# Aatricks/LightDiffusion-Next

Measured on AMD Instinct MI355X. Metric: sampler it/s (UNet steps/sec) SD1.5 1024x1024 bs=1 bf16, higher is better.
Workload: dtype bf16

## Files before the change

include/ldx.h:

```cpp
#ifndef LDX_H
#define LDX_H
#include <stdint.h>
#ifdef __cplusplus
extern "C" {
#endif

#define LDX_OK 0
#define LDX_EINVAL (-1)
#define LDX_EMISSING (-2)
#define LDX_EHIP (-3)
#define LDX_ESTATE (-4)

#define LDX_BF16 0
#define LDX_F16 1
#define LDX_F32 2

typedef struct ldx_engine ldx_engine;

typedef struct ldx_unet_config {
    int32_t compute_dtype;
    int32_t in_channels;
    int32_t out_channels;
    int32_t model_channels;
    int32_t num_levels;
// ... 139 lines not shown
int ldx_op_mx_quant(const void* X, int ldx, int rows, int K, void* Y, int ldy, void* scales, int scales_ld, int dtype, void* stream);
int ldx_op_gemm_mx(const void* A8, int lda, const void* SA, int sa_ld, const void* W8, const void* SW, int sw_ld, int M, int N, int K,
                   const float* bias, int act, const void* R, int ldr, void* C, int ldc, float* Cf, int ldcf,
                   void* C8, int ldc8, void* SC, int sc_ld, int dtype, void* stream);
int ldx_op_gemm2(const void* A1, int lda1, const void* W1, int M1, int N1, int K1, const float* bias1, void* C1, int ldc1,
                 const void* A2, int lda2, const void* W2, int M2, int N2, int K2, const float* bias2, void* C2, int ldc2, int dtype, void* stream);
int ldx_op_gemm2_mx(const void* A1, int lda1, const void* SA1, int sa_ld1, const void* W1, const void* SW1, int sw_ld1, int M1, int N1, int K1,
                    const float* bias1, void* C1, int ldc1,
                    const void* A2, int lda2, const void* SA2, int sa_ld2, const void* W2, const void* SW2, int sw_ld2, int M2, int N2, int K2,
                    const float* bias2, void* C2, int ldc2, int dtype, void* stream);
int ldx_op_gemm_pick(int M, int N, int K, int mode, int geglu, int splitk, int f8, int c8, int ln_fold,
                     int Cin, int Hin, int Win, int Hout, int Wout, int stride, int M2, int N2, int K2,
                     int gn_hw, int gn_groups, int gn_max_chunks, int32_t* out);
int ldx_op_attn_pick(int B, int H, int Nq, int Mk, int D, int causal, int bias, int o8, int ldq, int ldk, int ldv, int ldo, int knorm_ws, int32_t* out);
int ldx_op_conv3x3(const void* X, int ldx, const void* W, int B, int Hin, int Win, int Cin, int Cout,
                   int stride, int Hout, int Wout, int resize_to_out, const float* bias,
                   const float* rowvec, int rowvec_ld, const void* R, int ldr, void* Y, int ldy,
                   int dtype, void* stream);
int ldx_op_conv3x3_skip(const void* X, int ldx, const void* X2, int ldx2, int Cin2, const void* W, int B, int H, int Wd, int Cin, int Cout,
                        const float* bias, void* Y, int ldy, int dtype, void* stream);
int ldx_op_groupnorm(const void* X, int ldx, void* Y, int ldy, int B, int HW, int C, int G, float eps, int silu,
                     const float* gamma, const float* beta, float* workspace, int dtype, void* stream);
int64_t ldx_op_groupnorm_workspace_floats(int B, int G);
int ldx_op_layernorm(const void* X, int ldx, void* Y, int ldy, int rows, int C, float eps,
                     const float* gamma, const float* beta, int dtype, void* stream);
int ldx_op_attention(const void* Q, int ldq, const void* K, int ldk, const void* V, int ldv, void* O, int ldo,
                     int B, int H, int Nq, int Mk, int D, float scale, int causal, int dtype, void* stream);
int ldx_op_xattn_block(void* H, int ldh, int64_t M, int N, int C, int heads, const float* ln_gamma, const float* ln_beta, float eps,
                       const void* Wq, const void* Wo, const float* bo, const void* K, int ldk, const void* V, int ldv, int Mk,
                       float scale, int dtype, void* stream);
int ldx_op_ff_block(void* H, int ldh, int64_t M, int C, int inner, const float* ln_gamma, const float* ln_beta, float eps,
                    const void* W1, const float* b1, const void* W2, const float* b2, int dtype, void* stream);
int ldx_op_rowgemm(const void* X, int ldx, void* Y, int ldy, int64_t M, int N, int K, const void* W, const float* bias, const void* R, int ldr,
                   int pro, const float* gamma, const float* beta, float eps, const float* partial, int nchunk, int HW, int dtype, void* stream);
int ldx_op_attention_bias(const void* Q, int ldq, const void* K, int ldk, const void* V, int ldv, void* O, int ldo,
                          int B, int H, int Nq, int Mk, int D, float scale, const float* bias, int bias_ld,
                          int64_t bias_head_stride, int dtype, void* stream);
int ldx_op_skinny(const float* x, int ldx, const void* W, const float* bias, float* out, int ldo,
                  int M, int N, int K, int in_act, int out_act, int dtype, void* stream);

#ifdef __cplusplus
}
#endif
#endif
```

lightdiffusion-next_amd/csrc/capi.cpp:

```cpp
#include <cstring>
#include <mutex>
#include <new>

#include "engine.h"

using namespace ldx;

struct ldx_engine { Engine* impl; };

#define GUARD_BEGIN try {
#define GUARD_END                                                                  \
    }                                                                              \
    catch (const std::bad_alloc&) { set_error("out of host memory"); return LDX_EINVAL; } \
    catch (const std::exception& ex) { set_error(std::string("internal error: ") + ex.what()); return LDX_EINVAL; }

static int check_device(int device) {
    int n = 0;
    if (hipGetDeviceCount(&n) != hipSuccess || n <= 0) { set_error("no HIP device available (libldx has no CPU fallback)"); return LDX_EHIP; }
    if (device < 0 || device >= n) { set_error("device ordinal out of range"); return LDX_EINVAL; }
    return LDX_OK;
}
static inline DType dtype_of(int d) { return d == LDX_F16 ? DT_F16 : DT_BF16; }
static int check_launch(const char* what) {
    hipError_t e = hipGetLastError();
// ... 515 lines not shown
    return check_launch("ldx_op_conv3x3");
}
int ldx_op_conv3x3_skip(const void* X, int ldx_, const void* X2, int ldx2, int Cin2, const void* W, int B, int H, int Wd, int Cin, int Cout,
                        const float* bias, void* Y, int ldy, int dtype, void* stream) {
    if (!X || !X2 || !W || !Y || Cin % 64 || Cin2 % 64 || ldx_ % 8 || ldx2 % 8 || B <= 0 || H <= 0 || Wd <= 0) {
        set_error("ldx_op_conv3x3_skip: bad argument (Cin % 64, Cin2 % 64)"); return LDX_EINVAL; }
    GemmArgs g{};
    g.A = X; g.lda = ldx_; g.W = W; g.M = B * H * Wd; g.N = Cout; g.K = 9 * Cin + Cin2; g.mode = 1;
    g.Cin = Cin; g.Hin = H; g.Win = Wd; g.Hout = H; g.Wout = Wd; g.stride = 1; g.Hv = H; g.Wv = Wd; g.resize = 0;
    g.A2 = X2; g.lda2 = ldx2; g.Cin2 = Cin2;
    g.bias = bias; g.rows_per_batch = H * Wd; g.C = Y; g.ldc = ldy;
    if (int rc = attach_splitk(g)) return rc;
    launch_gemm(g, dtype_of(dtype), (hipStream_t)stream);
    return check_launch("ldx_op_conv3x3_skip");
}
int64_t ldx_op_groupnorm_workspace_floats(int B, int G) { return (int64_t)B * GN_NCHUNK * G * 2; }
int ldx_op_groupnorm(const void* X, int ldx_, void* Y, int ldy, int B, int HW, int C, int G, float eps, int silu,
                     const float* gamma, const float* beta, float* workspace, int dtype, void* stream) {
    if (!X || !Y || !gamma || !beta || !workspace || C % 8 || C % G || G > 32 || ldx_ % 8 || ldy % 8) { set_error("ldx_op_groupnorm: bad argument"); return LDX_EINVAL; }
    GroupNormArgs a{X, ldx_, Y, ldy, B, HW, C, G, eps, silu, gamma, beta, workspace};
    launch_groupnorm(a, dtype_of(dtype), (hipStream_t)stream);
    return check_launch("ldx_op_groupnorm");
}
int ldx_op_layernorm(const void* X, int ldx_, void* Y, int ldy, int rows, int C, float eps, const float* gamma, const float* beta, int dtype, void* stream) {
    if (!X || !Y || !gamma || !beta || C % 8 || C > 4096) { set_error("ldx_op_layernorm: bad argument (C % 8, C <= 4096)"); return LDX_EINVAL; }
    LayerNormArgs a{X, ldx_, Y, ldy, rows, C, eps, gamma, beta};
    launch_layernorm(a, dtype_of(dtype), (hipStream_t)stream);
    return check_launch("ldx_op_layernorm");
}
int ldx_op_attention(const void* Q, int ldq, const void* K, int ldk, const void* V, int ldv, void* O, int ldo, int B, int H, int Nq, int Mk, int D,
                     float scale, int causal, int dtype, void* stream) {
    if (!Q || !K || !V || !O || D % 8 || (D > 160 && D != 512) || D <= 0 || ldq % 8 || ldk % 8 || ldv % 8 || ldo % 4 || Mk <= 0) { set_error("ldx_op_attention: bad argument (D % 8, D <= 160 or D == 512)"); return LDX_EINVAL; }
    AttnArgs a{Q, ldq, K, ldk, V, ldv, O, ldo, B, H, Nq, Mk, D, scale, causal, nullptr, 0, 0};
    const AttnPick p = attn_pick(a);
    if (D == 512 && p.family != AF_ATTN512) { set_error("ldx_op_attention: D = 512 without a mask only (attn512.hip)"); return LDX_EINVAL; }
    if (p.nsplit_want > 1) {
        a.nsplit = p.nsplit_want;
        a.split_ws = op_workspace(attn512_ws_floats(a, a.nsplit));
        if (!a.split_ws) { set_error("attention split workspace allocation failed"); return LDX_EHIP; }
    }
    if (attn_pipe_ok(a)) a.knorm_ws = op_workspace((size_t)B * H * ((Mk + 63) / 64));
    launch_attention(a, dtype_of(dtype), (hipStream_t)stream);
    return check_launch("ldx_op_attention");
}
int ldx_op_xattn_block(void* H, int ldh, int64_t M, int N, int C, int heads, const float* ln_gamma, const float* ln_beta, float eps,
                       const void* Wq, const void* Wo, const float* bo, const void* K, int ldk, const void* V, int ldv, int Mk,
// ... 45 lines not shown
```

lightdiffusion-next_amd/csrc/ldx_kernels.h:

```cpp
#pragma once
#include <hip/hip_runtime.h>
#include <stdint.h>

namespace ldx {

enum DType : int { DT_BF16 = 0, DT_F16 = 1 };

struct DevOnce { unsigned long long mask = 0; };
inline void set_dyn_lds(DevOnce& once, const void* fn, int bytes) {
    int dev = 0;
    (void)hipGetDevice(&dev);
    const unsigned long long bit = 1ull << (dev & 63);
    if (__atomic_load_n(&once.mask, __ATOMIC_RELAXED) & bit) return;
    (void)hipFuncSetAttribute(fn, hipFuncAttributeMaxDynamicSharedMemorySize, bytes);
    __atomic_fetch_or(&once.mask, bit, __ATOMIC_RELAXED);
}

struct GemmArgs {
    const void* A;  int lda;
    const void* W;
    int M, N, K;
    int mode;
    int Cin, Hin, Win;
    int Hv, Wv;
// ... 117 lines not shown
    float* gn_out; int gn_nchunk;
    int abl;
    long dup_rows;
};
bool rowgemm_ok(const RowGemmArgs& a);
void launch_rowgemm(const RowGemmArgs& a, DType dt, hipStream_t s);
bool xattn_block_ok(const XAttnArgs& a);
void launch_xattn_block(const XAttnArgs& a, DType dt, hipStream_t s);

struct GroupNormArgs {
    const void* X; int ldx; void* Y; int ldy;
    int B, HW, C, G; float eps; int silu;
    const float* gamma; const float* beta;
    float* partial;
    int nchunk;
    int stats_chunks;
};
constexpr int GN_NCHUNK = 256;
constexpr int GN_FOLD = 64;
constexpr int GN_MAX_PRODUCER_CHUNKS = 32768;
static inline size_t gn_workspace_rows(long HWmax) { long r = HWmax / 64; if (r < GN_NCHUNK) r = GN_NCHUNK; if (r > GN_MAX_PRODUCER_CHUNKS) r = GN_MAX_PRODUCER_CHUNKS; return (size_t)r; }
void launch_groupnorm(const GroupNormArgs& a, DType dt, hipStream_t s);
bool gn_uses_small_kernel(int B, long HW, int C, int G);

struct LayerNormArgs {
    const void* X; int ldx; void* Y; int ldy; int rows, C; float eps;
    const float* gamma; const float* beta;
    const float* scale; const float* shift; int mod_ld; int rows_per_batch;
    int rms;
    void* Y8; int ldy8; uint32_t* S8; int s8_ld;
};
void launch_layernorm(const LayerNormArgs& a, DType dt, hipStream_t s);

struct PrepArgs {
    const float* x; const float* sigma; int B, C, H, W; int Cpad; void* xc;
    const float* log_sigmas; int n_sigmas; const float* temb_table; int temb_dim;
    float* temb_out; float* t_out;
    int scale_input;
    const float* t_in;
    int xB;
    const float* cc; int Cx;
    const float* emb_table; int emb_n; float* emb_out;
};
void launch_prep(const PrepArgs& a, DType dt, hipStream_t s);
void launch_timestep(const float* sigma, const float* log_sigmas, int n_sigmas, int n, int* out, hipStream_t s);
struct FinishArgs { const float* eps; int ld; const float* x; const float* sigma; float* out; int B, C, HW; int xB; };
// ... 61 lines not shown
```

lightdiffusion-next_amd/csrc/norm.hip:

```cpp
#include <stdlib.h>
#include "ldx_device.h"
#include "ldx_kernels.h"

namespace ldx {

struct GnGeom { int CH, TX, RY; };
static inline GnGeom gn_geom(int C) {
    const int cpp = C / 8;
    int ch = 1;
    while (ch < 4 && (cpp / ch > 256 || cpp % ch)) ch *= 2;
    GnGeom g; g.CH = ch; g.TX = cpp / ch; g.RY = 256 / g.TX; if (g.RY < 1) g.RY = 1;
    return g;
}

template <typename T, int CH>
__global__ __launch_bounds__(256) void gn_stats_kernel(const GroupNormArgs p, int TX, int RY) {
    extern __shared__ float sred[];
    const int tid = threadIdx.x;
    const int tx = tid % TX, ty = tid / TX;
    const int b = blockIdx.y, chunk = blockIdx.x;
    const int per = (p.HW + p.nchunk - 1) / p.nchunk;
    const int pb = chunk * per, pe = min(p.HW, pb + per);
    const T* __restrict__ X = (const T*)p.X + (long)b * p.HW * p.ldx;

    float s[CH][8], q[CH][8];
#pragma unroll
    for (int k = 0; k < CH; ++k)
#pragma unroll
        for (int e = 0; e < 8; ++e) { s[k][e] = 0.f; q[k][e] = 0.f; }

    if (ty < RY) {
        int pix = pb + ty;
        for (; pix + 3 * RY < pe; pix += 4 * RY) {
            uint4 u[4][CH];
#pragma unroll
            for (int r = 0; r < 4; ++r)
#pragma unroll
                for (int k = 0; k < CH; ++k) u[r][k] = *(const uint4*)(X + (long)(pix + r * RY) * p.ldx + (tx + TX * k) * 8);
#pragma unroll
            for (int r = 0; r < 4; ++r)
#pragma unroll
                for (int k = 0; k < CH; ++k) {
                    float f[8];
                    unpack8<T>(u[r][k], f);
#pragma unroll
                    for (int e = 0; e < 8; ++e) { s[k][e] += f[e]; q[k][e] = fmaf(f[e], f[e], q[k][e]); }
                }
        }
        for (; pix < pe; pix += RY) {
#pragma unroll
            for (int k = 0; k < CH; ++k) {
                float f[8];
                unpack8<T>(*(const uint4*)(X + (long)pix * p.ldx + (tx + TX * k) * 8), f);
#pragma unroll
                for (int e = 0; e < 8; ++e) { s[k][e] += f[e]; q[k][e] = fmaf(f[e], f[e], q[k][e]); }
            }
        }
#pragma unroll
        for (int k = 0; k < CH; ++k)
#pragma unroll
            for (int e = 0; e < 8; ++e) {
                const int c = (tx + TX * k) * 8 + e;
                sred[(ty * p.C + c) * 2 + 0] = s[k][e];
                sred[(ty * p.C + c) * 2 + 1] = q[k][e];
            }
    }
    __syncthreads();
    if (tid < p.G * 2) {
        const int g = tid >> 1, st = tid & 1;
        const int cpg = p.C / p.G;
        float acc = 0.f;
        for (int r = 0; r < RY; ++r)
            for (int c = g * cpg; c < (g + 1) * cpg; ++c) acc += sred[(r * p.C + c) * 2 + st];
        p.partial[(((long)b * p.nchunk + chunk) * p.G + g) * 2 + st] = acc;
    }
}

template <typename T, int CH>
__global__ __launch_bounds__(256) void gn_apply_kernel(const GroupNormArgs p, int TX, int RY, int nblk) {
    __shared__ float smean[64], srstd[64];
    __shared__ float sred[8][32][2];
    const int tid = threadIdx.x;
    const int b = blockIdx.y;
    const int cpg = p.C / p.G;
    const int tx = tid % TX, ty = tid / TX;
    const bool act = ty < RY;
    const T* __restrict__ X = (const T*)p.X + (long)b * p.HW * p.ldx;
    T* __restrict__ Y = (T*)p.Y + (long)b * p.HW * p.ldy;
    const int per = (p.HW + nblk - 1) / nblk;
    const int pb = blockIdx.x * per, pe = min(p.HW, pb + per);
    int pix = pb + ty;
    uint4 u0[4][CH];
    const bool first4 = act && pix + 3 * RY < pe;
    if (first4) {
#pragma unroll
        for (int r = 0; r < 4; ++r)
#pragma unroll
            for (int k = 0; k < CH; ++k) u0[r][k] = *(const uint4*)(X + (long)(pix + r * RY) * p.ldx + (tx + TX * k) * 8);
    }
    float4 gam[CH][2], bet[CH][2];
    if (act) {
#pragma unroll
        for (int k = 0; k < CH; ++k) {
            const int c = (tx + TX * k) * 8;
            gam[k][0] = *(const float4*)(p.gamma + c); gam[k][1] = *(const float4*)(p.gamma + c + 4);
            bet[k][0] = *(const float4*)(p.beta + c);  bet[k][1] = *(const float4*)(p.beta + c + 4);
        }
    }
    {
        const int g = tid & 31, sl = tid >> 5;
        float su = 0.f, sq = 0.f;
        if (g < p.G) {
            const float2* pp = (const float2*)p.partial + ((long)b * p.nchunk) * p.G + g;
            int ck = sl;
            for (; ck + 120 < p.nchunk; ck += 128) {
                float2 v[16];
#pragma unroll
                for (int u = 0; u < 16; ++u) v[u] = pp[(long)(ck + 8 * u) * p.G];
#pragma unroll
                for (int u = 0; u < 16; ++u) { su += v[u].x; sq += v[u].y; }
            }
            for (; ck + 56 < p.nchunk; ck += 64) {
                float2 v[8];
#pragma unroll
                for (int u = 0; u < 8; ++u) v[u] = pp[(long)(ck + 8 * u) * p.G];
#pragma unroll
                for (int u = 0; u < 8; ++u) { su += v[u].x; sq += v[u].y; }
            }
            for (; ck < p.nchunk; ck += 8) { const float2 v = pp[(long)ck * p.G]; su += v.x; sq += v.y; }
        }
        sred[sl][g][0] = su; sred[sl][g][1] = sq;
    }
    __syncthreads();
    if (tid < p.G) {
        float su = 0.f, sq = 0.f;
#pragma unroll
        for (int sl = 0; sl < 8; ++sl) { su += sred[sl][tid][0]; sq += sred[sl][tid][1]; }
        const float n = (float)p.HW * (float)cpg;
        const float mean = su / n;
        const float var = fmaxf(sq / n - mean * mean, 0.f);
        smean[tid] = mean;
        srstd[tid] = rsqrtf(var + p.eps);
    }
    __syncthreads();
    if (!act) return;
    float sc[CH][8], sh[CH][8];
#pragma unroll
    for (int k = 0; k < CH; ++k) {
        const float ga[8] = {gam[k][0].x, gam[k][0].y, gam[k][0].z, gam[k][0].w, gam[k][1].x, gam[k][1].y, gam[k][1].z, gam[k][1].w};
        const float be[8] = {bet[k][0].x, bet[k][0].y, bet[k][0].z, bet[k][0].w, bet[k][1].x, bet[k][1].y, bet[k][1].z, bet[k][1].w};
#pragma unroll
        for (int e = 0; e < 8; ++e) {
            const int c = (tx + TX * k) * 8 + e;
            const int g = c / cpg;
            const float a = srstd[g] * ga[e];
            sc[k][e] = a;
            sh[k][e] = be[e] - smean[g] * a;
        }
    }
    auto emit = [&](const uint4& u, const int pix, const int k) __attribute__((always_inline)) {
        float f[8];
        unpack8<T>(u, f);
#pragma unroll
        for (int e = 0; e < 8; ++e) {
            float y = fmaf(f[e], sc[k][e], sh[k][e]);
            if (p.silu) y = silu_f(y);
            f[e] = y;
        }
        *(uint4*)(Y + (long)pix * p.ldy + (tx + TX * k) * 8) = pack8<T>(f);
    };
    if (first4) {
#pragma unroll
        for (int r = 0; r < 4; ++r)
#pragma unroll
            for (int k = 0; k < CH; ++k) emit(u0[r][k], pix + r * RY, k);
        pix += 4 * RY;
    }
    for (; pix + 3 * RY < pe; pix += 4 * RY) {
        uint4 u[4][CH];
#pragma unroll
        for (int r = 0; r < 4; ++r)
#pragma unroll
            for (int k = 0; k < CH; ++k) u[r][k] = *(const uint4*)(X + (long)(pix + r * RY) * p.ldx + (tx + TX * k) * 8);
#pragma unroll
        for (int r = 0; r < 4; ++r)
#pragma unroll
            for (int k = 0; k < CH; ++k) emit(u[r][k], pix + r * RY, k);
    }
    for (; pix < pe; pix += RY) {
#pragma unroll
        for (int k = 0; k < CH; ++k) emit(*(const uint4*)(X + (long)pix * p.ldx + (tx + TX * k) * 8), pix, k);
    }
}

template <typename T>
__global__ __launch_bounds__(256) void gn_small_kernel(const GroupNormArgs p) {
    __shared__ float red[2][4];
    const int tid = threadIdx.x, g = blockIdx.x, b = blockIdx.y;
    const int cpg = p.C / p.G, cpc = cpg >> 3;
    const long total = (long)p.HW * cpc;
    const T* __restrict__ X = (const T*)p.X + (long)b * p.HW * p.ldx + g * cpg;
    T* __restrict__ Y = (T*)p.Y + (long)b * p.HW * p.ldy + g * cpg;
    float su = 0.f, sq = 0.f;
    constexpr int KMAX = 12;
    if (total <= (long)KMAX * 256) {
        uint4 u[KMAX]; int px[KMAX], cc[KMAX];
#pragma unroll
        for (int k = 0; k < KMAX; ++k) {
            const long ii = (long)tid + 256 * k;
            px[k] = (int)(ii / cpc); cc[k] = (int)(ii % cpc);
            u[k] = ii < total ? *(const uint4*)(X + (long)px[k] * p.ldx + cc[k] * 8) : make_uint4(0u, 0u, 0u, 0u);
        }
#pragma unroll
        for (int k = 0; k < KMAX; ++k) {
            if ((long)tid + 256 * k < total) {
                float f[8];
                unpack8<T>(u[k], f);
#pragma unroll
                for (int e = 0; e < 8; ++e) { su += f[e]; sq = fmaf(f[e], f[e], sq); }
            }
        }
        su = wave_sum(su); sq = wave_sum(sq);
        if ((tid & 63) == 0) { red[0][tid >> 6] = su; red[1][tid >> 6] = sq; }
        __syncthreads();
        const float n = (float)p.HW * (float)cpg;
        const float mean = ((red[0][0] + red[0][1]) + (red[0][2] + red[0][3])) / n;
        const float var = fmaxf(((red[1][0] + red[1][1]) + (red[1][2] + red[1][3])) / n - mean * mean, 0.f);
        const float rstd = rsqrtf(var + p.eps);
#pragma unroll
        for (int k = 0; k < KMAX; ++k) {
            if ((long)tid + 256 * k < total) {
                float f[8];
                unpack8<T>(u[k], f);
                const float* gm = p.gamma + g * cpg + cc[k] * 8;
                const float* bt = p.beta + g * cpg + cc[k] * 8;
                const float4 g0 = *(const float4*)gm, g1 = *(const float4*)(gm + 4), b0 = *(const float4*)bt, b1 = *(const float4*)(bt + 4);
                const float gg[8] = {g0.x, g0.y, g0.z, g0.w, g1.x, g1.y, g1.z, g1.w}, bb[8] = {b0.x, b0.y, b0.z, b0.w, b1.x, b1.y, b1.z, b1.w};
#pragma unroll
                for (int e = 0; e < 8; ++e) {
                    const float a = rstd * gg[e];
                    float y = fmaf(f[e], a, bb[e] - mean * a);
                    if (p.silu) y = silu_f(y);
                    f[e] = y;
                }
                *(uint4*)(Y + (long)px[k] * p.ldy + cc[k] * 8) = pack8<T>(f);
            }
        }
        return;
    }
    long i = tid;
    for (; i + 3 * 256 < total; i += 4 * 256) {
        uint4 u[4];
#pragma unroll
        for (int r = 0; r < 4; ++r) {
            const long ii = i + r * 256;
            const int pix = (int)(ii / cpc), ch = (int)(ii % cpc);
            u[r] = *(const uint4*)(X + (long)pix * p.ldx + ch * 8);
        }
#pragma unroll
        for (int r = 0; r < 4; ++r) {
            float f[8];
            unpack8<T>(u[r], f);
#pragma unroll
            for (int e = 0; e < 8; ++e) { su += f[e]; sq = fmaf(f[e], f[e], sq); }
        }
    }
    for (; i < total; i += 256) {
        const int pix = (int)(i / cpc), ch = (int)(i % cpc);
        float f[8];
        unpack8<T>(*(const uint4*)(X + (long)pix * p.ldx + ch * 8), f);
#pragma unroll
        for (int e = 0; e < 8; ++e) { su += f[e]; sq = fmaf(f[e], f[e], sq); }
    }
    su = wave_sum(su); sq = wave_sum(sq);
    if ((tid & 63) == 0) { red[0][tid >> 6] = su; red[1][tid >> 6] = sq; }
    __syncthreads();
    const float n = (float)p.HW * (float)cpg;
    const float mean = ((red[0][0] + red[0][1]) + (red[0][2] + red[0][3])) / n;
    const float var = fmaxf(((red[1][0] + red[1][1]) + (red[1][2] + red[1][3])) / n - mean * mean, 0.f);
    const float rstd = rsqrtf(var + p.eps);
    auto emit = [&](const uint4& u, const int pix, const int ch) __attribute__((always_inline)) {
        float f[8];
        unpack8<T>(u, f);
        const float* gm = p.gamma + g * cpg + ch * 8;
        const float* bt = p.beta + g * cpg + ch * 8;
        const float4 g0 = *(const float4*)gm, g1 = *(const float4*)(gm + 4), b0 = *(const float4*)bt, b1 = *(const float4*)(bt + 4);
        const float gg[8] = {g0.x, g0.y, g0.z, g0.w, g1.x, g1.y, g1.z, g1.w}, bb[8] = {b0.x, b0.y, b0.z, b0.w, b1.x, b1.y, b1.z, b1.w};
#pragma unroll
        for (int e = 0; e < 8; ++e) {
            const float a = rstd * gg[e];
            float y = fmaf(f[e], a, bb[e] - mean * a);
            if (p.silu) y = silu_f(y);
            f[e] = y;
        }
        *(uint4*)(Y + (long)pix * p.ldy + ch * 8) = pack8<T>(f);
    };
    i = tid;
    for (; i + 3 * 256 < total; i += 4 * 256) {
        uint4 u[4]; int px[4], cc[4];
#pragma unroll
        for (int r = 0; r < 4; ++r) {
            const long ii = i + r * 256;
            px[r] = (int)(ii / cpc); cc[r] = (int)(ii % cpc);
            u[r] = *(const uint4*)(X + (long)px[r] * p.ldx + cc[r] * 8);
        }
#pragma unroll
        for (int r = 0; r < 4; ++r) emit(u[r], px[r], cc[r]);
    }
    for (; i < total; i += 256) {
        const int pix = (int)(i / cpc), ch = (int)(i % cpc);
// ... 2 lines not shown
}

__global__ __launch_bounds__(64) void gn_fold_kernel(const float* in, float* out, int n_in, int G) {
    const int f = blockIdx.x, b = blockIdx.y, t = threadIdx.x;
    if (t >= G * 2) return;
    const int per = (n_in + GN_FOLD - 1) / GN_FOLD;
    const int lo = f * per, hi = min(n_in, lo + per);
    float a0 = 0.f, a1 = 0.f, a2 = 0.f, a3 = 0.f;
    int c = lo;
    for (; c + 3 < hi; c += 4) {
        const float v0 = in[((long)b * n_in + c) * G * 2 + t], v1 = in[((long)b * n_in + c + 1) * G * 2 + t];
        const float v2 = in[((long)b * n_in + c + 2) * G * 2 + t], v3 = in[((long)b * n_in + c + 3) * G * 2 + t];
        a0 += v0; a1 += v1; a2 += v2; a3 += v3;
    }
    for (; c < hi; ++c) a0 += in[((long)b * n_in + c) * G * 2 + t];
    out[((long)b * GN_FOLD + f) * G * 2 + t] = (a0 + a1) + (a2 + a3);
}

bool gn_uses_small_kernel(int B, long HW, int C, int G) {
    static const long small_max = getenv("LDX_GN_SMALL_MAX") ? atol(getenv("LDX_GN_SMALL_MAX")) : 256 * 80;
    return G > 0 && (C / G) % 8 == 0 && HW * (C / G) <= small_max && (long)G * B >= 32;
}

template <typename T>
static void launch_gn_t(const GroupNormArgs& a_in, hipStream_t s) {
    GroupNormArgs a = a_in;
    if (a.stats_chunks > 0) {
        const GnGeom g = gn_geom(a.C);
        a.nchunk = a.stats_chunks;
        if (a.stats_chunks > GN_NCHUNK) {
            float* folded = a.partial + (size_t)a.B * a.stats_chunks * a.G * 2;
            hipLaunchKernelGGL(gn_fold_kernel, dim3(GN_FOLD, a.B), dim3(64), 0, s, a.partial, folded, a.stats_chunks, a.G);
            a.partial = folded; a.nchunk = GN_FOLD;
        }
        int nblk = (a.HW + g.RY * 8 - 1) / (g.RY * 8);
        if (nblk > 512) nblk = 512;
        if (nblk < 1) nblk = 1;
        dim3 grid2(nblk, a.B);
        switch (g.CH) {
            case 1: hipLaunchKernelGGL((gn_apply_kernel<T, 1>), grid2, dim3(256), 0, s, a, g.TX, g.RY, nblk); break;
            case 2: hipLaunchKernelGGL((gn_apply_kernel<T, 2>), grid2, dim3(256), 0, s, a, g.TX, g.RY, nblk); break;
            default: hipLaunchKernelGGL((gn_apply_kernel<T, 4>), grid2, dim3(256), 0, s, a, g.TX, g.RY, nblk); break;
        }
        return;
    }
    if (gn_uses_small_kernel(a.B, a.HW, a.C, a.G)) {
        hipLaunchKernelGGL((gn_small_kernel<T>), dim3(a.G, a.B), dim3(256), 0, s, a);
        return;
    }
    const GnGeom g = gn_geom(a.C);
    int nchunk = (1024 + a.B - 1) / a.B;
    const int maxc = (a.HW + g.RY * 4 - 1) / (g.RY * 4);
    if (nchunk > maxc) nchunk = maxc;
    if (nchunk > GN_NCHUNK) nchunk = GN_NCHUNK;
    if (nchunk < 1) nchunk = 1;
    a.nchunk = nchunk;
    dim3 grid1(nchunk, a.B);
    const size_t lds = (size_t)g.RY * a.C * 2 * sizeof(float);
    int nblk = (a.HW + g.RY * 8 - 1) / (g.RY * 8);
    if (nblk > 512) nblk = 512;
    if (nblk < 1) nblk = 1;
    dim3 grid2(nblk, a.B);
    switch (g.CH) {
        case 1:
            hipLaunchKernelGGL((gn_stats_kernel<T, 1>), grid1, dim3(256), lds, s, a, g.TX, g.RY);
            hipLaunchKernelGGL((gn_apply_kernel<T, 1>), grid2, dim3(256), 0, s, a, g.TX, g.RY, nblk);
            break;
        case 2:
            hipLaunchKernelGGL((gn_stats_kernel<T, 2>), grid1, dim3(256), lds, s, a, g.TX, g.RY);
            hipLaunchKernelGGL((gn_apply_kernel<T, 2>), grid2, dim3(256), 0, s, a, g.TX, g.RY, nblk);
            break;
        default:
            hipLaunchKernelGGL((gn_stats_kernel<T, 4>), grid1, dim3(256), lds, s, a, g.TX, g.RY);
            hipLaunchKernelGGL((gn_apply_kernel<T, 4>), grid2, dim3(256), 0, s, a, g.TX, g.RY, nblk);
            break;
    }
}

void launch_groupnorm(const GroupNormArgs& a, DType dt, hipStream_t s) {
    if (dt == DT_BF16) launch_gn_t<__bf16>(a, s); else launch_gn_t<_Float16>(a, s);
}

template <typename T, int LPR, int NCH>
__global__ __launch_bounds__(256) void ln_kernel(const LayerNormArgs p) {
    constexpr int RPW = 64 / LPR;
    const int lane = threadIdx.x & 63, sub = lane % LPR;
    const long row_raw = ((long)blockIdx.x * 4 + (threadIdx.x >> 6)) * RPW + lane / LPR;
    const bool live = row_raw < p.rows;
    const long row = live ? row_raw : p.rows - 1;
    const int nch = p.C >> 3;
    const T* __restrict__ x = (const T*)p.X + row * p.ldx;
    T* __restrict__ y = (T*)p.Y + row * p.ldy;
    float f[NCH][8];
    float sum = 0.f;
    uint4 raw[NCH];
#pragma unroll
    for (int i = 0; i < NCH; ++i) { const int ch = sub + LPR * i; raw[i] = *(const uint4*)(x + (ch < nch ? ch : 0) * 8); }
#pragma unroll
    for (int i = 0; i < NCH; ++i) {
// ... 124 lines not shown
```

lightdiffusion-next_amd/lib.py:

```python
import ctypes as C
import os

_HERE = os.path.dirname(os.path.abspath(__file__))
LIB_PATH = os.path.join(_HERE, "libldx.so")

LDX_BF16, LDX_F16, LDX_F32 = 0, 1, 2


class LdxError(RuntimeError):
    pass


class ldx_unet_config(C.Structure):
    _fields_ = [
        ("compute_dtype", C.c_int32),
        ("in_channels", C.c_int32),
        ("out_channels", C.c_int32),
        ("model_channels", C.c_int32),
        ("num_levels", C.c_int32),
        ("channel_mult", C.c_int32 * 8),
        ("num_res_blocks", C.c_int32 * 8),
        ("transformer_depth", C.c_int32 * 32),
        ("transformer_depth_output", C.c_int32 * 48),
        ("transformer_depth_middle", C.c_int32),
# ... 59 lines not shown
    "ldx_clip_encode": (_i, [_vp, _vp, _i, _i, _i, _vp, _vp, _vp]),
    "ldx_clip_pooled": (_i, [_vp, _vp, _vp, _i, _i, _i, _vp, _vp]),
    "ldx_clip_set_extra_embeddings": (_i, [_vp, _vp, _i]),
    "ldx_flux_fbcache": (_i, [_vp, _f]),
    "ldx_flux_set_fp8": (_i, [_vp, _i]),
    "ldx_flux_fbcache_stats": (_i, [_vp, C.POINTER(_i64), C.POINTER(_i64)]),
    "ldx_esrgan_create": (_i, [C.POINTER(ldx_esrgan_config), _i, C.POINTER(_vp)]),
    "ldx_esrgan_forward": (_i, [_vp, _vp, _i, _i, _i, _vp, _vp]),
    "ldx_tile_blend": (_i, [_vp, _i, _i, _vp, _vp, _i, _i, _i, _i, _i, _i, _vp]),
    "ldx_tile_finish": (_i, [_vp, _vp, _i64, _i, _vp]),
    "ldx_t5_create": (_i, [C.POINTER(ldx_t5_config), _i, C.POINTER(_vp)]),
    "ldx_t5_encode": (_i, [_vp, _vp, _i, _i, _vp, _vp, _vp]),
    "ldx_flux_create": (_i, [C.POINTER(ldx_flux_config), _i, C.POINTER(_vp)]),
    "ldx_flux_forward": (_i, [_vp, _vp, _vp, _vp, _vp, _vp, _vp, _vp, _i, _i, _i, _i, _i, _vp, _vp]),
    "ldx_sampler_step": (_i, [_i, _vp, _vp, _vp, _vp, _i64, _f, _f, _f, _vp]),
    "ldx_bislerp_pass": (_i, [_vp, _vp, _i, _i, _i, _i, _i, _i, _vp, _vp, _vp, _vp]),
    "ldx_vae_encode": (_i, [_vp, _vp, _i, _i, _i, _vp, _vp]),
    "ldx_bilinear": (_i, [_vp, _vp, _i, _i, _i, _i, _i, _vp]),
    "ldx_op_convert": (_i, [_vp, _vp, _i64, _i, _i, _vp]),
    "ldx_op_gemm": (_i, [_vp, _i, _vp, _i, _i, _i, _vp, _vp, _i, _i, _i, _vp, _i, _vp, _i, _vp, _i, _i, _vp]),
    "ldx_op_conv3x3": (_i, [_vp, _i, _vp, _i, _i, _i, _i, _i, _i, _i, _i, _i, _vp, _vp, _i, _vp, _i, _vp, _i, _i, _vp]),
    "ldx_op_groupnorm": (_i, [_vp, _i, _vp, _i, _i, _i, _i, _i, _f, _i, _vp, _vp, _vp, _i, _vp]),
    "ldx_op_groupnorm_workspace_floats": (_i64, [_i, _i]),
    "ldx_op_conv3x3_skip": (_i, [_vp, _i, _vp, _i, _i, _vp, _i, _i, _i, _i, _i, _vp, _vp, _i, _i, _vp]),
    "ldx_op_layernorm_mx": (_i, [_vp, _i, _i, _i, _f, _vp, _vp, _vp, _i, _vp, _i, _i, _vp]),
    "ldx_op_attention_mx": (_i, [_vp, _i, _vp, _i, _vp, _i, _vp, _i, _vp, _i, _i, _i, _i, _i, _f, _i, _vp]),
    "ldx_op_qk_norm_rope_mx": (_i, [_vp, _i, _i, _i, _i, _vp, _vp, _vp, _vp, _f, _vp, _vp, _i, _vp, _vp, _i, _i, _vp]),
    "ldx_op_mx_vt_quant": (_i, [_vp, _i, _i, _i, _i, _vp, _vp, _i, _i, _vp]),
    "ldx_op_attention_fp8": (_i, [_vp, _i, _vp, _i, _vp, _i, _vp, _i, _vp, _vp, _i, _vp, _i, _vp, _i, _vp, _i, _i, _i, _i, _i, _f, _i, _vp]),
    "ldx_op_mx_quant": (_i, [_vp, _i, _i, _i, _vp, _i, _vp, _i, _i, _vp]),
    "ldx_op_gemm2": (_i, [_vp, _i, _vp, _i, _i, _i, _vp, _vp, _i, _vp, _i, _vp, _i, _i, _i, _vp, _vp, _i, _i, _vp]),
    "ldx_op_gemm2_mx": (_i, [_vp, _i, _vp, _i, _vp, _vp, _i, _i, _i, _i, _vp, _vp, _i, _vp, _i, _vp, _i, _vp, _vp, _i, _i, _i, _i, _vp, _vp, _i, _i, _vp]),
    "ldx_op_gemm_pick": (_i, [_i] * 21 + [C.POINTER(C.c_int32)]),
    "ldx_op_attn_pick": (_i, [_i] * 13 + [C.POINTER(C.c_int32)]),
    "ldx_op_gemm_mx": (_i, [_vp, _i, _vp, _i, _vp, _vp, _i, _i, _i, _i, _vp, _i, _vp, _i, _vp, _i, _vp, _i, _vp, _i, _vp, _i, _i, _vp]),
    "ldx_op_layernorm": (_i, [_vp, _i, _vp, _i, _i, _i, _f, _vp, _vp, _i, _vp]),
    "ldx_op_attention": (_i, [_vp, _i, _vp, _i, _vp, _i, _vp, _i, _i, _i, _i, _i, _i, _f, _i, _i, _vp]),
    "ldx_op_xattn_block": (_i, [_vp, _i, _i64, _i, _i, _i, _vp, _vp, _f, _vp, _vp, _vp, _vp, _i, _vp, _i, _i, _f, _i, _vp]),
    "ldx_op_ff_block": (_i, [_vp, _i, _i64, _i, _i, _vp, _vp, _f, _vp, _vp, _vp, _vp, _i, _vp]),
    "ldx_op_rowgemm": (_i, [_vp, _i, _vp, _i, _i64, _i, _i, _vp, _vp, _vp, _i, _i, _vp, _vp, _f, _vp, _i, _i, _i, _vp]),
    "ldx_op_attention_bias": (_i, [_vp, _i, _vp, _i, _vp, _i, _vp, _i, _i, _i, _i, _i, _i, _f, _vp, _i, _i64, _i, _vp]),
    "ldx_op_skinny": (_i, [_vp, _i, _vp, _vp, _vp, _i, _i, _i, _i, _i, _i, _i, _vp]),
}
EXPORTS = tuple(_SIGS)

_lib = None
# ... 39 lines not shown
```

Baseline: 75.37.

## Restructure GroupNorm stats/apply kernels with double-buffered loads and occupancy-aware grid

The GroupNorm apply kernel now double-buffers row loads (ua/ub), starting the next loads before emitting the current ones, and overlaps the partial-stat fold with the first data loads. The stats kernel uses a CH-dependent load depth with clamped tail loads, and waves_per_eu hints are set per channel width. The apply grid is sized from an assumed CU count of 256 and 4 workgroups per CU rather than a fixed 512 cap. The small kernel stages gamma and beta in LDS. New C API entry points expose the apply pass with caller-supplied partials, which adds surface area and hardcodes hardware assumptions.

```diff
diff --git a/include/ldx.h b/include/ldx.h
--- a/include/ldx.h
+++ b/include/ldx.h
@@ -185,6 +185,9 @@
 int ldx_op_groupnorm(const void* X, int ldx, void* Y, int ldy, int B, int HW, int C, int G, float eps, int silu,
                      const float* gamma, const float* beta, float* workspace, int dtype, void* stream);
 int64_t ldx_op_groupnorm_workspace_floats(int B, int G);
+int ldx_op_groupnorm_nchunk(int B, int HW, int C, int G);
+int ldx_op_groupnorm_apply(const void* X, int ldx, void* Y, int ldy, int B, int HW, int C, int G, float eps, int silu,
+                           const float* gamma, const float* beta, const float* partial, int nchunk, int dtype, void* stream);
 int ldx_op_layernorm(const void* X, int ldx, void* Y, int ldy, int rows, int C, float eps,
                      const float* gamma, const float* beta, int dtype, void* stream);
 int ldx_op_attention(const void* Q, int ldq, const void* K, int ldk, const void* V, int ldv, void* O, int ldo,
diff --git a/lightdiffusion-next_amd/csrc/capi.cpp b/lightdiffusion-next_amd/csrc/capi.cpp
--- a/lightdiffusion-next_amd/csrc/capi.cpp
+++ b/lightdiffusion-next_amd/csrc/capi.cpp
@@ -561,6 +561,19 @@
     launch_groupnorm(a, dtype_of(dtype), (hipStream_t)stream);
     return check_launch("ldx_op_groupnorm");
 }
+int ldx_op_groupnorm_nchunk(int B, int HW, int C, int G) {
+    if (B <= 0 || HW <= 0 || C <= 0 || G <= 0 || C % 8 || C % G) return 0;
+    return gn_uses_small_kernel(B, HW, C, G) ? 0 : gn_stats_nchunk(B, HW, C);
+}
+int ldx_op_groupnorm_apply(const void* X, int ldx_, void* Y, int ldy, int B, int HW, int C, int G, float eps, int silu,
+                           const float* gamma, const float* beta, const float* partial, int nchunk, int dtype, void* stream) {
+    if (!X || !Y || !gamma || !beta || !partial || C % 8 || C % G || G > 32 || ldx_ % 8 || ldy % 8 || B <= 0 || HW <= 0 || nchunk < 1 || nchunk > GN_NCHUNK) {
+        set_error("ldx_op_groupnorm_apply: bad argument (1 <= nchunk <= 256)"); return LDX_EINVAL; }
+    GroupNormArgs a{X, ldx_, Y, ldy, B, HW, C, G, eps, silu, gamma, beta, const_cast<float*>(partial)};
+    a.stats_chunks = nchunk;
+    launch_groupnorm(a, dtype_of(dtype), (hipStream_t)stream);
+    return check_launch("ldx_op_groupnorm_apply");
+}
 int ldx_op_layernorm(const void* X, int ldx_, void* Y, int ldy, int rows, int C, float eps, const float* gamma, const float* beta, int dtype, void* stream) {
     if (!X || !Y || !gamma || !beta || C % 8 || C > 4096) { set_error("ldx_op_layernorm: bad argument (C % 8, C <= 4096)"); return LDX_EINVAL; }
     LayerNormArgs a{X, ldx_, Y, ldy, rows, C, eps, gamma, beta};
diff --git a/lightdiffusion-next_amd/csrc/ldx_kernels.h b/lightdiffusion-next_amd/csrc/ldx_kernels.h
--- a/lightdiffusion-next_amd/csrc/ldx_kernels.h
+++ b/lightdiffusion-next_amd/csrc/ldx_kernels.h
@@ -163,6 +163,7 @@
 static inline size_t gn_workspace_rows(long HWmax) { long r = HWmax / 64; if (r < GN_NCHUNK) r = GN_NCHUNK; if (r > GN_MAX_PRODUCER_CHUNKS) r = GN_MAX_PRODUCER_CHUNKS; return (size_t)r; }
 void launch_groupnorm(const GroupNormArgs& a, DType dt, hipStream_t s);
 bool gn_uses_small_kernel(int B, long HW, int C, int G);
+int gn_stats_nchunk(int B, long HW, int C);
 
 struct LayerNormArgs {
     const void* X; int ldx; void* Y; int ldy; int rows, C; float eps;
diff --git a/lightdiffusion-next_amd/csrc/norm.hip b/lightdiffusion-next_amd/csrc/norm.hip
--- a/lightdiffusion-next_amd/csrc/norm.hip
+++ b/lightdiffusion-next_amd/csrc/norm.hip
@@ -4,6 +4,7 @@
 
 namespace ldx {
 
+constexpr int GN_SMALL_CPG = 256;
 struct GnGeom { int CH, TX, RY; };
 static inline GnGeom gn_geom(int C) {
     const int cpp = C / 8;
@@ -13,9 +14,27 @@
     return g;
 }
 
+template <int CH> struct GnDepth {
+    static constexpr int D = 4;
+    static constexpr int SD = CH == 1 ? 8 : CH == 2 ? 5 : 4;
+    static constexpr int APPLY_WAVES = CH == 1 ? 7 : CH == 2 ? 4 : 2, STATS_WAVES = CH == 1 ? 8 : CH == 2 ? 5 : 3;
+};
+
+template <typename T, int CH, int D>
+__device__ __forceinline__ void gn_load_rows(uint4 (&u)[D][CH], const T* __restrict__ X, int pix, int pe, int RY, int ldx, int tx, int TX) {
+#pragma unroll
+    for (int r = 0; r < D; ++r) {
+        const int pr = min(pix + r * RY, pe - 1);
+#pragma unroll
+        for (int k = 0; k < CH; ++k) u[r][k] = *(const uint4*)(X + (long)pr * ldx + (tx + TX * k) * 8);
+    }
+}
+
 template <typename T, int CH>
-__global__ __launch_bounds__(256) void gn_stats_kernel(const GroupNormArgs p, int TX, int RY) {
+__global__ __launch_bounds__(256) __attribute__((amdgpu_waves_per_eu(GnDepth<CH>::STATS_WAVES, GnDepth<CH>::STATS_WAVES)))
+void gn_stats_kernel(const GroupNormArgs p, int TX, int RY) {
     extern __shared__ float sred[];
+    constexpr int D = GnDepth<CH>::SD;
     const int tid = threadIdx.x;
     const int tx = tid % TX, ty = tid / TX;
     const int b = blockIdx.y, chunk = blockIdx.x;
@@ -30,30 +49,20 @@
         for (int e = 0; e < 8; ++e) { s[k][e] = 0.f; q[k][e] = 0.f; }
 
     if (ty < RY) {
-        int pix = pb + ty;
-        for (; pix + 3 * RY < pe; pix += 4 * RY) {
-            uint4 u[4][CH];
-#pragma unroll
-            for (int r = 0; r < 4; ++r)
-#pragma unroll
-                for (int k = 0; k < CH; ++k) u[r][k] = *(const uint4*)(X + (long)(pix + r * RY) * p.ldx + (tx + TX * k) * 8);
-#pragma unroll
-            for (int r = 0; r < 4; ++r)
-#pragma unroll
-                for (int k = 0; k < CH; ++k) {
-                    float f[8];
-                    unpack8<T>(u[r][k], f);
-#pragma unroll
-                    for (int e = 0; e < 8; ++e) { s[k][e] += f[e]; q[k][e] = fmaf(f[e], f[e], q[k][e]); }
+        for (int pix = pb + ty; pix < pe; pix += D * RY) {
+            uint4 u[D][CH];
+            gn_load_rows<T, CH, D>(u, X, pix, pe, RY, p.ldx, tx, TX);
+#pragma unroll
+            for (int r = 0; r < D; ++r) {
+                if (pix + r * RY < pe) {
+#pragma unroll
+                    for (int k = 0; k < CH; ++k) {
+                        float f[8];
+                        unpack8<T>(u[r][k], f);
+#pragma unroll
+                        for (int e = 0; e < 8; ++e) { s[k][e] += f[e]; q[k][e] = fmaf(f[e], f[e], q[k][e]); }
+                    }
                 }
-        }
-        for (; pix < pe; pix += RY) {
-#pragma unroll
-            for (int k = 0; k < CH; ++k) {
-                float f[8];
-                unpack8<T>(*(const uint4*)(X + (long)pix * p.ldx + (tx + TX * k) * 8), f);
-#pragma unroll
-                for (int e = 0; e < 8; ++e) { s[k][e] += f[e]; q[k][e] = fmaf(f[e], f[e], q[k][e]); }
             }
         }
 #pragma unroll
@@ -69,67 +78,81 @@
     if (tid < p.G * 2) {
         const int g = tid >> 1, st = tid & 1;
         const int cpg = p.C / p.G;
+        const int n = RY * cpg;
         float acc = 0.f;
-        for (int r = 0; r < RY; ++r)
-            for (int c = g * cpg; c < (g + 1) * cpg; ++c) acc += sred[(r * p.C + c) * 2 + st];
+        int r = 0, cc = 0, i = 0;
+        auto next = [&]() __attribute__((always_inline)) {
+            const float v = sred[(r * p.C + g * cpg + cc) * 2 + st];
+            if (++cc == cpg) { cc = 0; ++r; }
+            return v;
+        };
+        for (; i + 8 <= n; i += 8) {
+            float v[8];
+#pragma unroll
+            for (int u = 0; u < 8; ++u) v[u] = next();
+#pragma unroll
+            for (int u = 0; u < 8; ++u) acc += v[u];
+        }
+        for (; i < n; ++i) acc += next();
         p.partial[(((long)b * p.nchunk + chunk) * p.G + g) * 2 + st] = acc;
     }
 }
 
+template <int N>
+__device__ __forceinline__ void gn_fold_load(float2 (&v)[16], const float2* __restrict__ pp, int G, int nchunk, int row0) {
+#pragma unroll
+    for (int j = 0; j < N; ++j) v[j] = pp[(long)min(row0 + 8 * j, nchunk - 1) * G];
+}
+template <int N>
+__device__ __forceinline__ void gn_fold_add(const float2 (&v)[16], int nchunk, int row0, float& su, float& sq) {
+#pragma unroll
+    for (int j = 0; j < N; ++j)
+        if (row0 + 8 * j < nchunk) { su += v[j].x; sq += v[j].y; }
+}
+
 template <typename T, int CH>
-__global__ __launch_bounds__(256) void gn_apply_kernel(const GroupNormArgs p, int TX, int RY, int nblk) {
+__global__ __launch_bounds__(256) __attribute__((amdgpu_waves_per_eu(GnDepth<CH>::APPLY_WAVES, GnDepth<CH>::APPLY_WAVES)))
+void gn_apply_kernel(const GroupNormArgs p, int TX, int RY, int per) {
     __shared__ float smean[64], srstd[64];
     __shared__ float sred[8][32][2];
+    constexpr int D = GnDepth<CH>::D;
     const int tid = threadIdx.x;
     const int b = blockIdx.y;
     const int cpg = p.C / p.G;
     const int tx = tid % TX, ty = tid / TX;
-    const bool act = ty < RY;
     const T* __restrict__ X = (const T*)p.X + (long)b * p.HW * p.ldx;
     T* __restrict__ Y = (T*)p.Y + (long)b * p.HW * p.ldy;
-    const int per = (p.HW + nblk - 1) / nblk;
     const int pb = blockIdx.x * per, pe = min(p.HW, pb + per);
     int pix = pb + ty;
-    uint4 u0[4][CH];
-    const bool first4 = act && pix + 3 * RY < pe;
-    if (first4) {
-#pragma unroll
-        for (int r = 0; r < 4; ++r)
-#pragma unroll
-            for (int k = 0; k < CH; ++k) u0[r][k] = *(const uint4*)(X + (long)(pix + r * RY) * p.ldx + (tx + TX * k) * 8);
-    }
+    const bool act = ty < RY && pix < pe;
+    const int h = D * RY;
+    const int ltx = act ? tx : 0, lTX = act ? TX : 0, lRY = act ? RY : 0, lpix = act ? pix : pb, lpe = act ? pe : pb + 1;
+    const int fg = min(tid & 31, p.G - 1), fsl = tid >> 5;
+    const float2* pp = (const float2*)p.partial + ((long)b * p.nchunk) * p.G + fg;
+    float2 pv[16];
+    if (p.nchunk <= 8) gn_fold_load<1>(pv, pp, p.G, p.nchunk, fsl);
+    else if (p.nchunk <= 64) gn_fold_load<8>(pv, pp, p.G, p.nchunk, fsl);
+    else gn_fold_load<16>(pv, pp, p.G, p.nchunk, fsl);
     float4 gam[CH][2], bet[CH][2];
-    if (act) {
+    uint4 ua[D][CH], ub[D][CH];
+    gn_load_rows<T, CH, D>(ua, X, lpix, lpe, lRY, p.ldx, ltx, lTX);
+    {
+        float su = 0.f, sq = 0.f;
+        if (p.nchunk <= 8) gn_fold_add<1>(pv, p.nchunk, fsl, su, sq);
+        else if (p.nchunk <= 64) gn_fold_add<8>(pv, p.nchunk, fsl, su, sq);
+        else gn_fold_add<16>(pv, p.nchunk, fsl, su, sq);
+        if (p.nchunk > 128) {
+            gn_fold_load<16>(pv, pp, p.G, p.nchunk, fsl + 128);
+            gn_fold_add<16>(pv, p.nchunk, fsl + 128, su, sq);
+        }
+        gn_load_rows<T, CH, D>(ub, X, lpix + D * lRY, lpe, lRY, p.ldx, ltx, lTX);
 #pragma unroll
         for (int k = 0; k < CH; ++k) {
-            const int c = (tx + TX * k) * 8;
+            const int c = (ltx + lTX * k) * 8;
             gam[k][0] = *(const float4*)(p.gamma + c); gam[k][1] = *(const float4*)(p.gamma + c + 4);
             bet[k][0] = *(const float4*)(p.beta + c);  bet[k][1] = *(const float4*)(p.beta + c + 4);
         }
-    }
-    {
-        const int g = tid & 31, sl = tid >> 5;
-        float su = 0.f, sq = 0.f;
-        if (g < p.G) {
-            const float2* pp = (const float2*)p.partial + ((long)b * p.nchunk) * p.G + g;
-            int ck = sl;
-            for (; ck + 120 < p.nchunk; ck += 128) {
-                float2 v[16];
-#pragma unroll
-                for (int u = 0; u < 16; ++u) v[u] = pp[(long)(ck + 8 * u) * p.G];
-#pragma unroll
-                for (int u = 0; u < 16; ++u) { su += v[u].x; sq += v[u].y; }
-            }
-            for (; ck + 56 < p.nchunk; ck += 64) {
-                float2 v[8];
-#pragma unroll
-                for (int u = 0; u < 8; ++u) v[u] = pp[(long)(ck + 8 * u) * p.G];
-#pragma unroll
-                for (int u = 0; u < 8; ++u) { su += v[u].x; sq += v[u].y; }
-            }
-            for (; ck < p.nchunk; ck += 8) { const float2 v = pp[(long)ck * p.G]; su += v.x; sq += v.y; }
-        }
-        sred[sl][g][0] = su; sred[sl][g][1] = sq;
+        sred[fsl][tid & 31][0] = su; sred[fsl][tid & 31][1] = sq;
     }
     __syncthreads();
     if (tid < p.G) {
@@ -147,57 +170,78 @@
     float sc[CH][8], sh[CH][8];
 #pragma unroll
     for (int k = 0; k < CH; ++k) {
+        const int c0 = (tx + TX * k) * 8;
         const float ga[8] = {gam[k][0].x, gam[k][0].y, gam[k][0].z, gam[k][0].w, gam[k][1].x, gam[k][1].y, gam[k][1].z, gam[k][1].w};
         const float be[8] = {bet[k][0].x, bet[k][0].y, bet[k][0].z, bet[k][0].w, bet[k][1].x, bet[k][1].y, bet[k][1].z, bet[k][1].w};
 #pragma unroll
         for (int e = 0; e < 8; ++e) {
-            const int c = (tx + TX * k) * 8 + e;
-            const int g = c / cpg;
+            const int g = (c0 + e) / cpg;
             const float a = srstd[g] * ga[e];
             sc[k][e] = a;
             sh[k][e] = be[e] - smean[g] * a;
         }
     }
-    auto emit = [&](const uint4& u, const int pix, const int k) __attribute__((always_inline)) {
-        float f[8];
-        unpack8<T>(u, f);
-#pragma unroll
-        for (int e = 0; e < 8; ++e) {
-            float y = fmaf(f[e], sc[k][e], sh[k][e]);
-            if (p.silu) y = silu_f(y);
-            f[e] = y;
-        }
-        *(uint4*)(Y + (long)pix * p.ldy + (tx + TX * k) * 8) = pack8<T>(f);
-    };
-    if (first4) {
-#pragma unroll
-        for (int r = 0; r < 4; ++r)
-#pragma unroll
-            for (int k = 0; k < CH; ++k) emit(u0[r][k], pix + r * RY, k);
-        pix += 4 * RY;
-    }
-    for (; pix + 3 * RY < pe; pix += 4 * RY) {
-        uint4 u[4][CH];
-#pragma unroll
-        for (int r = 0; r < 4; ++r)
-#pragma unroll
-            for (int k = 0; k < CH; ++k) u[r][k] = *(const uint4*)(X + (long)(pix + r * RY) * p.ldx + (tx + TX * k) * 8);
-#pragma unroll
-        for (int r = 0; r < 4; ++r)
-#pragma unroll
-            for (int k = 0; k < CH; ++k) emit(u[r][k], pix + r * RY, k);
-    }
-    for (; pix < pe; pix += RY) {
-#pragma unroll
-        for (int k = 0; k < CH; ++k) emit(*(const uint4*)(X + (long)pix * p.ldx + (tx + TX * k) * 8), pix, k);
-    }
+    auto emit_row = [&](const uint4 (&u)[CH], const int row) __attribute__((always_inline)) {
+#pragma unroll
+        for (int k = 0; k < CH; ++k) {
+            float f[8];
+            unpack8<T>(u[k], f);
+#pragma unroll
+            for (int e = 0; e < 8; ++e) {
+                float y = fmaf(f[e], sc[k][e], sh[k][e]);
+                if (p.silu) y = silu_f(y);
+                f[e] = y;
+            }
+            *(uint4*)(Y + (long)row * p.ldy + (tx + TX * k) * 8) = pack8<T>(f);
+        }
+    };
+    auto emit_full = [&](const uint4 (&u)[D][CH], const int pix) __attribute__((always_inline)) {
+#pragma unroll
+        for (int r = 0; r < D; ++r) emit_row(u[r], pix + r * RY);
+    };
+    auto emit_tail = [&](const uint4 (&u)[D][CH], const int pix) __attribute__((always_inline)) {
+#pragma unroll
+        for (int r = 0; r < D; ++r)
+            if (pix + r * RY < pe) emit_row(u[r], pix + r * RY);
+    };
+    while (pix + 2 * h < pe) {
+        emit_full(ua, pix);
+        gn_load_rows<T, CH, D>(ua, X, pix + 2 * h, pe, RY, p.ldx, tx, TX);
+        emit_full(ub, pix + h);
+        gn_load_rows<T, CH, D>(ub, X, pix + 3 * h, pe, RY, p.ldx, tx, TX);
+        pix += 2 * h;
+    }
+    emit_tail(ua, pix);
+    emit_tail(ub, pix + h);
 }
 
 template <typename T>
 __global__ __launch_bounds__(256) void gn_small_kernel(const GroupNormArgs p) {
     __shared__ float red[2][4];
+    __shared__ __attribute__((aligned(16))) float sgb[2][GN_SMALL_CPG];
     const int tid = threadIdx.x, g = blockIdx.x, b = blockIdx.y;
     const int cpg = p.C / p.G, cpc = cpg >> 3;
+    const bool staged = cpg <= GN_SMALL_CPG;
+    auto request_gb = [&](float& gv, float& bv) __attribute__((always_inline)) {
+        gv = 0.f; bv = 0.f;
+        if (staged && tid < cpg) { gv = p.gamma[g * cpg + tid]; bv = p.beta[g * cpg + tid]; }
+    };
+    auto park_gb = [&](const float gv, const float bv) __attribute__((always_inline)) {
+        if (staged && tid < cpg) { sgb[0][tid] = gv; sgb[1][tid] = bv; }
+    };
+    auto affine8 = [&](const int ch, float (&gg)[8], float (&bb)[8]) __attribute__((always_inline)) {
+        float4 g0, g1, b0, b1;
+        if (staged) {
+            g0 = *(const float4*)&sgb[0][ch * 8]; g1 = *(const float4*)&sgb[0][ch * 8 + 4];
+            b0 = *(const float4*)&sgb[1][ch * 8]; b1 = *(const float4*)&sgb[1][ch * 8 + 4];
+        } else {
+            const float* gm = p.gamma + g * cpg + ch * 8;
+            const float* bt = p.beta + g * cpg + ch * 8;
+            g0 = *(const float4*)gm; g1 = *(const float4*)(gm + 4); b0 = *(const float4*)bt; b1 = *(const float4*)(bt + 4);
+        }
+        gg[0] = g0.x; gg[1] = g0.y; gg[2] = g0.z; gg[3] = g0.w; gg[4] = g1.x; gg[5] = g1.y; gg[6] = g1.z; gg[7] = g1.w;
+        bb[0] = b0.x; bb[1] = b0.y; bb[2] = b0.z; bb[3] = b0.w; bb[4] = b1.x; bb[5] = b1.y; bb[6] = b1.z; bb[7] = b1.w;
+    };
     const long total = (long)p.HW * cpc;
     const T* __restrict__ X = (const T*)p.X + (long)b * p.HW * p.ldx + g * cpg;
     T* __restrict__ Y = (T*)p.Y + (long)b * p.HW * p.ldy + g * cpg;
@@ -211,6 +255,8 @@
             px[k] = (int)(ii / cpc); cc[k] = (int)(ii % cpc);
             u[k] = ii < total ? *(const uint4*)(X + (long)px[k] * p.ldx + cc[k] * 8) : make_uint4(0u, 0u, 0u, 0u);
         }
+        float gv, bv;
+        request_gb(gv, bv);
 #pragma unroll
         for (int k = 0; k < KMAX; ++k) {
             if ((long)tid + 256 * k < total) {
@@ -222,6 +268,7 @@
         }
         su = wave_sum(su); sq = wave_sum(sq);
         if ((tid & 63) == 0) { red[0][tid >> 6] = su; red[1][tid >> 6] = sq; }
+        park_gb(gv, bv);
         __syncthreads();
         const float n = (float)p.HW * (float)cpg;
         const float mean = ((red[0][0] + red[0][1]) + (red[0][2] + red[0][3])) / n;
@@ -232,10 +279,8 @@
             if ((long)tid + 256 * k < total) {
                 float f[8];
                 unpack8<T>(u[k], f);
-                const float* gm = p.gamma + g * cpg + cc[k] * 8;
-                const float* bt = p.beta + g * cpg + cc[k] * 8;
-                const float4 g0 = *(const float4*)gm, g1 = *(const float4*)(gm + 4), b0 = *(const float4*)bt, b1 = *(const float4*)(bt + 4);
-                const float gg[8] = {g0.x, g0.y, g0.z, g0.w, g1.x, g1.y, g1.z, g1.w}, bb[8] = {b0.x, b0.y, b0.z, b0.w, b1.x, b1.y, b1.z, b1.w};
+                float gg[8], bb[8];
+                affine8(cc[k], gg, bb);
 #pragma unroll
                 for (int e = 0; e < 8; ++e) {
                     const float a = rstd * gg[e];
@@ -248,6 +293,8 @@
         }
         return;
     }
+    float gv, bv;
+    request_gb(gv, bv);
     long i = tid;
     for (; i + 3 * 256 < total; i += 4 * 256) {
         uint4 u[4];
@@ -274,6 +321,7 @@
     }
     su = wave_sum(su); sq = wave_sum(sq);
     if ((tid & 63) == 0) { red[0][tid >> 6] = su; red[1][tid >> 6] = sq; }
+    park_gb(gv, bv);
     __syncthreads();
     const float n = (float)p.HW * (float)cpg;
     const float mean = ((red[0][0] + red[0][1]) + (red[0][2] + red[0][3])) / n;
@@ -282,10 +330,8 @@
     auto emit = [&](const uint4& u, const int pix, const int ch) __attribute__((always_inline)) {
         float f[8];
         unpack8<T>(u, f);
-        const float* gm = p.gamma + g * cpg + ch * 8;
-        const float* bt = p.beta + g * cpg + ch * 8;
-        const float4 g0 = *(const float4*)gm, g1 = *(const float4*)(gm + 4), b0 = *(const float4*)bt, b1 = *(const float4*)(bt + 4);
-        const float gg[8] = {g0.x, g0.y, g0.z, g0.w, g1.x, g1.y, g1.z, g1.w}, bb[8] = {b0.x, b0.y, b0.z, b0.w, b1.x, b1.y, b1.z, b1.w};
+        float gg[8], bb[8];
+        affine8(ch, gg, bb);
 #pragma unroll
         for (int e = 0; e < 8; ++e) {
             const float a = rstd * gg[e];
@@ -334,6 +380,40 @@
     return G > 0 && (C / G) % 8 == 0 && HW * (C / G) <= small_max && (long)G * B >= 32;
 }
 
+constexpr int GN_WG_PER_CU = 4, GN_CUS = 256;
+static inline void gn_apply_grid(const GnGeom& g, int B, int HW, int& nblk, int& per) {
+    const int rows = 2 * 4 * g.RY;
+    const long nbuf = ((long)HW + rows - 1) / rows;
+    long cap = (long)GN_WG_PER_CU * GN_CUS / (B > 0 ? B : 1);
+    if (cap < 1) cap = 1;
+    const long bpw = (nbuf + cap - 1) / cap;
+    per = (int)(bpw * rows);
+    nblk = (int)((nbuf + bpw - 1) / bpw);
+    if (nblk < 1) nblk = 1;
+}
+
+int gn_stats_nchunk(int B, long HW, int C) {
+    const GnGeom g = gn_geom(C);
+    long nchunk = (1024 + B - 1) / B;
+    const long maxc = (HW + g.RY * 4 - 1) / (g.RY * 4);
+    if (nchunk > maxc) nchunk = maxc;
+    if (nchunk > GN_NCHUNK) nchunk = GN_NCHUNK;
+    if (nchunk < 1) nchunk = 1;
+    return (int)nchunk;
+}
+
+template <typename T>
+static void launch_gn_apply_t(const GroupNormArgs& a, const GnGeom& g, hipStream_t s) {
+    int nblk, per;
+    gn_apply_grid(g, a.B, a.HW, nblk, per);
+    dim3 grid2(nblk, a.B);
+    switch (g.CH) {
+        case 1: hipLaunchKernelGGL((gn_apply_kernel<T, 1>), grid2, dim3(256), 0, s, a, g.TX, g.RY, per); break;
+        case 2: hipLaunchKernelGGL((gn_apply_kernel<T, 2>), grid2, dim3(256), 0, s, a, g.TX, g.RY, per); break;
+        default: hipLaunchKernelGGL((gn_apply_kernel<T, 4>), grid2, dim3(256), 0, s, a, g.TX, g.RY, per); break;
+    }
+}
+
 template <typename T>
 static void launch_gn_t(const GroupNormArgs& a_in, hipStream_t s) {
     GroupNormArgs a = a_in;
@@ -345,15 +425,7 @@
             hipLaunchKernelGGL(gn_fold_kernel, dim3(GN_FOLD, a.B), dim3(64), 0, s, a.partial, folded, a.stats_chunks, a.G);
             a.partial = folded; a.nchunk = GN_FOLD;
         }
-        int nblk = (a.HW + g.RY * 8 - 1) / (g.RY * 8);
-        if (nblk > 512) nblk = 512;
-        if (nblk < 1) nblk = 1;
-        dim3 grid2(nblk, a.B);
-        switch (g.CH) {
-            case 1: hipLaunchKernelGGL((gn_apply_kernel<T, 1>), grid2, dim3(256), 0, s, a, g.TX, g.RY, nblk); break;
-            case 2: hipLaunchKernelGGL((gn_apply_kernel<T, 2>), grid2, dim3(256), 0, s, a, g.TX, g.RY, nblk); break;
-            default: hipLaunchKernelGGL((gn_apply_kernel<T, 4>), grid2, dim3(256), 0, s, a, g.TX, g.RY, nblk); break;
-        }
+        launch_gn_apply_t<T>(a, g, s);
         return;
     }
     if (gn_uses_small_kernel(a.B, a.HW, a.C, a.G)) {
@@ -361,32 +433,15 @@
         return;
     }
     const GnGeom g = gn_geom(a.C);
-    int nchunk = (1024 + a.B - 1) / a.B;
-    const int maxc = (a.HW + g.RY * 4 - 1) / (g.RY * 4);
-    if (nchunk > maxc) nchunk = maxc;
-    if (nchunk > GN_NCHUNK) nchunk = GN_NCHUNK;
-    if (nchunk < 1) nchunk = 1;
-    a.nchunk = nchunk;
-    dim3 grid1(nchunk, a.B);
+    a.nchunk = gn_stats_nchunk(a.B, a.HW, a.C);
+    dim3 grid1(a.nchunk, a.B);
     const size_t lds = (size_t)g.RY * a.C * 2 * sizeof(float);
-    int nblk = (a.HW + g.RY * 8 - 1) / (g.RY * 8);
-    if (nblk > 512) nblk = 512;
-    if (nblk < 1) nblk = 1;
-    dim3 grid2(nblk, a.B);
     switch (g.CH) {
-        case 1:
-            hipLaunchKernelGGL((gn_stats_kernel<T, 1>), grid1, dim3(256), lds, s, a, g.TX, g.RY);
-            hipLaunchKernelGGL((gn_apply_kernel<T, 1>), grid2, dim3(256), 0, s, a, g.TX, g.RY, nblk);
-            break;
-        case 2:
-            hipLaunchKernelGGL((gn_stats_kernel<T, 2>), grid1, dim3(256), lds, s, a, g.TX, g.RY);
-            hipLaunchKernelGGL((gn_apply_kernel<T, 2>), grid2, dim3(256), 0, s, a, g.TX, g.RY, nblk);
-            break;
-        default:
-            hipLaunchKernelGGL((gn_stats_kernel<T, 4>), grid1, dim3(256), lds, s, a, g.TX, g.RY);
-            hipLaunchKernelGGL((gn_apply_kernel<T, 4>), grid2, dim3(256), 0, s, a, g.TX, g.RY, nblk);
-            break;
-    }
+        case 1: hipLaunchKernelGGL((gn_stats_kernel<T, 1>), grid1, dim3(256), lds, s, a, g.TX, g.RY); break;
+        case 2: hipLaunchKernelGGL((gn_stats_kernel<T, 2>), grid1, dim3(256), lds, s, a, g.TX, g.RY); break;
+        default: hipLaunchKernelGGL((gn_stats_kernel<T, 4>), grid1, dim3(256), lds, s, a, g.TX, g.RY); break;
+    }
+    launch_gn_apply_t<T>(a, g, s);
 }
 
 void launch_groupnorm(const GroupNormArgs& a, DType dt, hipStream_t s) {
diff --git a/lightdiffusion-next_amd/lib.py b/lightdiffusion-next_amd/lib.py
--- a/lightdiffusion-next_amd/lib.py
+++ b/lightdiffusion-next_amd/lib.py
@@ -105,6 +105,8 @@
     "ldx_op_conv3x3": (_i, [_vp, _i, _vp, _i, _i, _i, _i, _i, _i, _i, _i, _i, _vp, _vp, _i, _vp, _i, _vp, _i, _i, _vp]),
     "ldx_op_groupnorm": (_i, [_vp, _i, _vp, _i, _i, _i, _i, _i, _f, _i, _vp, _vp, _vp, _i, _vp]),
     "ldx_op_groupnorm_workspace_floats": (_i64, [_i, _i]),
+    "ldx_op_groupnorm_nchunk": (_i, [_i, _i, _i, _i]),
+    "ldx_op_groupnorm_apply": (_i, [_vp, _i, _vp, _i, _i, _i, _i, _i, _f, _i, _vp, _vp, _vp, _i, _i, _vp]),
     "ldx_op_conv3x3_skip": (_i, [_vp, _i, _vp, _i, _i, _vp, _i, _i, _i, _i, _i, _vp, _vp, _i, _i, _vp]),
     "ldx_op_layernorm_mx": (_i, [_vp, _i, _i, _i, _f, _vp, _vp, _vp, _i, _vp, _i, _i, _vp]),
     "ldx_op_attention_mx": (_i, [_vp, _i, _vp, _i, _vp, _i, _vp, _i, _vp, _i, _i, _i, _i, _i, _f, _i, _vp]),
```

Result: no change. 75.45 (median of 6 runs) (+0.1%).
